# rockcarry/ffcnn

Measured on AMD Instinct MI355X. Metric: frames/sec yolo-fastest-1.1 @320x320 batch-64 per GPU (u8 BGR frames -> net_input's conversion in the first kernel -> full forward: conv stack + YOLO decode + NMS, boxes on rank 0), higher is better.
Workload: dtype f32

## Files before the change

ffcnn_amd/capi.py:

```python
import ctypes as C
import os
import subprocess

import numpy as np

HERE = os.path.dirname(os.path.abspath(__file__))
ROOT = os.path.dirname(HERE)
DATA = os.path.join(ROOT, "data")
CFG = os.path.join(DATA, "yolo-fastest-1.1.cfg")
WEIGHTS = os.path.join(DATA, "yolo-fastest-1.1.weights")

f32p = C.POINTER(C.c_float)


class FFGPU:
    MAX_DET = 128
    MERGE_LDS_SLOTS = 1024
    KEEP_ALL, COMPAT_V6, NO_GRAPH, NO_FUSE, HOST_DETS, SPLIT2, CONCURRENT, BF16_PW = 1, 2, 4, 8, 16, 32, 64, 128
    FEAT_FLAT, FEAT_MEAN, FEAT_MAX = 0, 1, 2
    POST_NONE, POST_SOFTMAX, POST_L2 = 0, 1, 2
    TOPK_MAX = 16
    RELABEL_KEEP_SCORE, RELABEL_LABEL_SCORE = 0, 1
    RELABEL_ENTRIES, RELABEL_MERGED = 0, 1
    K_AUTO, K_GENERIC, K_DW_STREAM, K_DW_LDS, K_PW_MFMA, K_PW_GEMM, _K6, K_DENSE_SMALL, K_IGEMM, K_PW_BF16, K_GROUP_THIN, K_PW_X3, K_CONV_X3, K_PW_X3T = range(14)
# ... 264 lines not shown
TRAIL_SLOT_DTYPE = np.dtype([("id", "<i4"), ("last", "<i4"), ("n", "<i4"), ("head", "<i4"), ("cx", "<i4"), ("cy", "<i4"), ("reserved", "<i4", (2,)),
                             ("ring", TRAIL_POINT_DTYPE, (32,))])
LABEL_DTYPE = np.dtype([("index", "<i4"), ("value", "<f4")])
TEXT_ITEM_DTYPE = np.dtype([("x", "<i4"), ("y", "<i4"), ("fg", "u1", (4,)), ("bg", "u1", (4,)), ("scale", "u1"), ("flags", "u1"), ("len", "u1"), ("reserved", "u1"),
                            ("text", "u1", (44,))])
SEG_ITEM_DTYPE = np.dtype([("x0", "<i4"), ("y0", "<i4"), ("x1", "<i4"), ("y1", "<i4"), ("color", "u1", (4,)), ("thickness", "u1"), ("dash", "u1"), ("flags", "u1"),
                           ("reserved", "u1"), ("reserved2", "<i4", (2,))])

EXPORTS = ["net_load", "net_free", "net_input", "net_forward", "net_dump", "net_profile", "groupconv",
           "ffgpu_device_count", "ffgpu_set_device", "ffgpu_last_error", "ffgpu_build_info",
           "ffgpu_net_weights_dev", "ffgpu_net_weights_commit",
           "ffgpu_exec_create", "ffgpu_exec_destroy", "ffgpu_exec_batch", "ffgpu_exec_arena_bytes",
           "ffgpu_exec_kernel_count", "ffgpu_exec_work_model", "ffgpu_exec_set_scale", "ffgpu_exec_forward_dev", "ffgpu_exec_forward_host",
           "ffgpu_exec_forward_bgr_dev", "ffgpu_exec_forward_bgr_frames_dev", "ffgpu_exec_forward_nv12_frames_dev", "ffgpu_exec_dets_dev", "ffgpu_exec_dets_host", "ffgpu_exec_set_ring", "ffgpu_exec_set_ring_strided", "ffgpu_exec_read_dets", "ffgpu_exec_read_layer", "ffgpu_exec_hash_layers",
           "ffgpu_exec_read_boxes", "ffgpu_exec_cand_capacity", "ffgpu_exec_graph_captures",
           "ffgpu_exec_profile", "ffgpu_exec_profile_steps", "ffgpu_exec_step_model", "ffgpu_groupconv_dev", "ffgpu_groupconv_kernel_name", "ffgpu_groupconv_time_dev", "ffgpu_irb_dev", "ffgpu_irb_flags_dev", "ffgpu_irb_plan_text", "ffgpu_irb_thin_launch_text", "ffgpu_irb_stage_plan_text", "ffgpu_front_plan_text", "ffgpu_irb_instantiations", "ffgpu_knobs_text", "ffgpu_dwpw_dev", "ffgpu_packed_records_bytes", "ffgpu_pack_records", "ffgpu_unpack_records",
           "ffgpu_shard_range", "ffgpu_node_create", "ffgpu_node_destroy", "ffgpu_node_ndev", "ffgpu_node_shard", "ffgpu_node_set_scale",
           "ffgpu_node_input_dev", "ffgpu_node_input_slot_dev", "ffgpu_node_depth", "ffgpu_node_rccl_ranks", "ffgpu_node_forward", "ffgpu_node_forward_host",
           "ffgpu_node_submit", "ffgpu_node_wait", "ffgpu_node_run",
           "ffgpu_merge_tiles_scratch_bytes", "ffgpu_merge_tiles_dev", "ffgpu_exec_merge_tiles", "ffgpu_exec_merged_dev", "ffgpu_exec_read_merged",
           "ffgpu_exec_read_merged_boxes", "ffgpu_tile_plan",
           "ffgpu_draw_boxes_bgr_dev", "ffgpu_draw_boxes_nv12_dev", "ffgpu_exec_draw_bgr", "ffgpu_exec_draw_nv12",
           "ffgpu_crop_table_bytes", "ffgpu_crop_slot_bytes", "ffgpu_crop_boxes_bgr_dev", "ffgpu_crop_boxes_nv12_dev", "ffgpu_exec_crop_bgr", "ffgpu_exec_crop_nv12",
           "ffgpu_crops_to_source_dev",
           "ffgpu_track_state_bytes", "ffgpu_track_reset_dev", "ffgpu_track_boxes_dev", "ffgpu_exec_track",
           "ffgpu_feature_dim", "ffgpu_exec_feature_dim", "ffgpu_features_dev", "ffgpu_exec_features", "ffgpu_topk_dev", "ffgpu_crops_relabel_dev",
           "ffgpu_exec_relabel",
           "ffgpu_match_workspace_bytes", "ffgpu_match_dev", "ffgpu_gallery_enroll_dev",
           "ffgpu_redact_boxes_bgr_dev", "ffgpu_redact_boxes_nv12_dev", "ffgpu_exec_redact_bgr", "ffgpu_exec_redact_nv12",
           "ffgpu_blur_boxes_bgr_dev", "ffgpu_blur_boxes_nv12_dev", "ffgpu_exec_blur_bgr", "ffgpu_exec_blur_nv12",
           "ffgpu_zones_state_bytes", "ffgpu_scene_check", "ffgpu_zones_reset_dev", "ffgpu_zones_boxes_dev", "ffgpu_exec_zones",
# ... 73 lines not shown
    L.ffgpu_exec_read_layer.argtypes = [vp, i, i, f32p, sz]
    L.ffgpu_exec_hash_layers.argtypes = [vp, vp, i]
    L.ffgpu_exec_profile.argtypes = [vp, vp, f32p]
    L.ffgpu_exec_profile_steps.argtypes = [vp, vp, C.POINTER(i), f32p, i]
    L.ffgpu_exec_step_model.argtypes = [vp, C.POINTER(i), C.POINTER(C.c_double), i]
    L.ffgpu_groupconv_dev.argtypes = [vp, vp, vp] + [i] * 15 + [vp]
    L.ffgpu_groupconv_kernel_name.restype = C.c_char_p
    L.ffgpu_groupconv_kernel_name.argtypes = [i] * 10
    L.ffgpu_groupconv_time_dev.restype = C.c_float
    L.ffgpu_groupconv_time_dev.argtypes = [vp, vp, vp] + [i] * 17 + [vp]
    L.ffgpu_irb_dev.restype = C.c_float
    L.ffgpu_irb_dev.argtypes = [vp] * 6 + [i] * 13 + [vp]
    L.ffgpu_irb_flags_dev.restype = C.c_float
    L.ffgpu_irb_flags_dev.argtypes = [vp] * 6 + [i] * 14 + [vp]
    L.ffgpu_irb_thin_launch_text.argtypes = [i] * 12 + [C.c_char_p, i]
    L.ffgpu_irb_plan_text.argtypes = [i] * 12 + [C.c_char_p, i]
    L.ffgpu_irb_stage_plan_text.argtypes = [i] * 7 + [C.c_char_p, i]
    L.ffgpu_front_plan_text.argtypes = [i] * 4 + [C.c_char_p, i]
    L.ffgpu_irb_instantiations.argtypes = [C.c_char_p, i]
    L.ffgpu_knobs_text.argtypes = [C.c_char_p, i]
    L.ffgpu_exec_read_boxes.argtypes = [vp, i, vp, i]
    L.ffgpu_exec_cand_capacity.argtypes = [vp]
    L.ffgpu_exec_graph_captures.argtypes = [vp]
    L.ffgpu_dwpw_dev.restype = C.c_float
    L.ffgpu_dwpw_dev.argtypes = [vp] * 4 + [i] * 10 + [vp]
    L.ffgpu_packed_records_bytes.restype = C.c_size_t
    L.ffgpu_packed_records_bytes.argtypes = [i, i]
    L.ffgpu_pack_records.restype = i
    L.ffgpu_pack_records.argtypes = [vp, i, C.c_long, i, i, vp, vp]
    L.ffgpu_shard_range.argtypes = [i, i, i, C.POINTER(i), C.POINTER(i)]
# ... 1308 lines not shown

def dwpw_dev(d_in, d_wd, d_wp, d_out, batch, iw, ih, c, oc, fs, actd=2, actp=0, warmup=0, iters=0, stream=None):
    us = lib().ffgpu_dwpw_dev(d_in, d_wd, d_wp, d_out, batch, iw, ih, c, oc, fs, actd, actp, warmup, iters, stream)
    if us < 0:
        raise RuntimeError("ffgpu_dwpw_dev failed: %s" % last_error())
    return us


def irb_thin_launch_text(shape, flags=0):
    buf = C.create_string_buffer(256)
    if lib().ffgpu_irb_thin_launch_text(*shape, flags, buf, len(buf)) < 0:
        raise RuntimeError("ffgpu_irb_thin_launch_text failed: %s" % last_error())
    return buf.value.decode()


def irb_dev(d_in, d_w1, d_wd, d_w2, d_res, d_out, batch, iw, ih, ic, ec, oc, stride, act1=2, actd=2, act2=0, res_act=0,
            warmup=0, iters=0, stream=None, flags=0):
    us = lib().ffgpu_irb_flags_dev(d_in, d_w1, d_wd, d_w2, d_res, d_out, batch, iw, ih, ic, ec, oc, stride, act1, actd, act2, res_act, flags,
                                   warmup, iters, stream)
    if us < 0:
        raise RuntimeError("ffgpu_irb_dev failed: %s" % last_error())
    return us


def preview_pane(src=None, dst=None):
    p = PreviewPane()
    if src is not None:
        p.sx, p.sy, p.sw, p.sh = (int(v) for v in src)
    if dst is not None:
        p.dx, p.dy, p.dw, p.dh = (int(v) for v in dst)
# ... 139 lines not shown
```

ffcnn_amd/csrc/ffgpu_conv_kernels.inc:

```
#include "ffgpu_dw_stream.inc"
#include "ffgpu_pw_mfma.inc"
#include "ffgpu_pw_gemm32.inc"
#include "ffgpu_pw_bf16.inc"
#include "ffgpu_conv_igemm.inc"
#include "ffgpu_dwpw.inc"
#include "ffgpu_conv_dense.inc"
#include "ffgpu_irb.inc"
#include "ffgpu_irb_thin.inc"
#include "ffgpu_front.inc"
#include "ffgpu_irb_wave.inc"
#include "ffgpu_irb_wave2.inc"
#include "ffgpu_irb_stage.inc"
#include "ffgpu_pw_x3.inc"
#include "ffgpu_pw_x3t.inc"
#include "ffgpu_conv_x3.inc"
#include "ffgpu_dw_lds.inc"
#include "ffgpu_dw_pair.inc"
#include "ffgpu_conv_thin.inc"

struct BareScratch {
    float *p = nullptr; size_t n = 0; int dev = -1;
    float *get(size_t need)
    {
        int d = 0;
// ... 1040 lines not shown
    if (f.ncp) { p.band = f.band; p.nbands = f.nbands; p.ntasks = f.ntasks; }
    for (const IrbThinKernel &k : irb_thin_kernels)
        if (k.IC == d.ic && k.OC == d.oc) return f.ncp ? k.pair(p, f, s) : k.launch(p, d.plan, s);
    ffgpu_set_error("irb_thin: no instantiation for %d -> 8 -> %d channels", d.ic, d.oc);
    return -1;
}

int ffgpu_irb_thin_launch_line(const IrbDesc &d, char *buf, size_t cap)
{
    if (d.plan.family != IRB_THIN) return snprintf(buf, cap, "unsupported");
    const ThinForm f = thin_form(d);
    char key[48];
    if (f.ncp) snprintf(key, sizeof key, "thin_pair<%d,8,%d,%d>", d.ic, d.oc, f.ncp);
    else snprintf(key, sizeof key, "thin<%d,8,%d>", d.ic, d.oc);
    return snprintf(buf, cap, "%s W=%d H=%d N=%d band=%d nbands=%d ntasks=%ld grid=%d block=256", key, d.W, d.H, d.N, f.band, f.nbands, f.ntasks, f.grid);
}

typedef int (*IrbwLaunch)(const IrbwP &, const IrbPlan &, hipStream_t);
struct IrbwKernel { int KS1, OT, S, NSI, NSO; bool big, x3, xl; Knob gate; IrbwLaunch launch; };
#define IRBW_K(ks1, ot, st, nsi, gate) \
    { ks1, ot, st, nsi, 1, true, false, false, gate, irb_launch_t<IrbwP, k_irbw<ks1, ot, st, nsi, true>> }, \
    { ks1, ot, st, nsi, 1, false, false, false, gate, irb_launch_t<IrbwP, k_irbw<ks1, ot, st, nsi, false>> }
static const IrbwKernel irbw_kernels[] = {
    { 2, 1, 1, 3, 2, true, true, false, K_NONE, irb_launch_t<IrbwP, k_irbw2<2, 3, true>> }, { 4, 1, 1, 3, 2, true, true, false, K_NONE, irb_launch_t<IrbwP, k_irbw2<4, 3, true>> },
    { 2, 1, 1, 3, 2, true, false, false, K_NONE, irb_launch_t<IrbwP, k_irbw2<2, 3, false>> }, { 4, 1, 1, 3, 2, true, false, false, K_NONE, irb_launch_t<IrbwP, k_irbw2<4, 3, false>> },
    { 12, 3, 1, 2, 1, true, true, true, K_NONE, irb_launch_t<IrbwP, k_irbw<12, 3, 1, 2, true, true, true>> },
    { 4, 2, 2, 4, 1, true, true, false, K_NONE, irb_launch_t<IrbwP, k_irbw<4, 2, 2, 4, true, true>> },
    { 6, 2, 1, 2, 1, true, true, false, K_NONE, irb_launch_t<IrbwP, k_irbw<6, 2, 1, 2, true, true>> },
    IRBW_K(1, 1, 1, 2, K_NONE), IRBW_K(2, 1, 1, 2, K_NONE), IRBW_K(4, 1, 1, 2, K_NONE), IRBW_K(2, 2, 1, 2, K_NONE), IRBW_K(4, 2, 1, 2, K_NONE),
    IRBW_K(6, 2, 1, 2, K_NONE), IRBW_K(12, 3, 1, 2, K_NONE), IRBW_K(1, 1, 2, 3, K_NONE), IRBW_K(2, 1, 2, 3, K_NONE), IRBW_K(4, 2, 2, 4, K_NONE),
// ... 480 lines not shown
                        key, p.N, p.H, p.W, p.OH, p.OW, p.ic, p.ec, p.oc, p.act1, p.actd, p.act2, p.res_act, p.TWq, p.TH, p.EW, p.EH, p.tiles_x, p.tiles_y, p.ntiles, p.ngroups, p.G, p.WPB,
                        p.o_w2, p.o_cs, p.cs_floats, p.xl_off, p.red_cap, p.in_elems, p.vec, p.half_last, p.m_ew, p.m_tx, p.m_ty, p.m_twq, p.xcd, c.lds, c.grid, c.block, c.half, c.pack_floats);
    }
    if (c.family == IRB_WG) {
        const IrbP p = irb_params(d);
        const IrbKernel &k = irb_kernels[c.inst];
        irb_key(k, key, sizeof key);
        return snprintf(buf, cap, "%s N=%d H=%d W=%d OH=%d OW=%d ic=%d ec=%d oc=%d stride=%d act=%g,%g,%g,%g tile=%d,%d,%d,%d,%d,%d NPin=%d NPout=%d tiles=%d,%d,%d "
                        "k4=%d nchunks=%d ECH=%d CH=%d KS=%d red_off=%d vec_store=%d resident=%d inv_nsi=%d lds=%d grid=%d block=%d half=%d pack=%d",
                        key, p.N, p.H, p.W, p.OH, p.OW, p.ic, p.ec, p.oc, p.stride, p.act1, p.actd, p.act2, p.res_act, p.TH, p.TW, p.TWq, p.NF, p.EH, p.EW,
                        p.NPin, p.NPout, p.tiles_x, p.tiles_y, p.ntiles, p.k4, p.nchunks, p.ECH, p.CH, p.KS, p.red_off, p.vec_store, p.resident, p.inv_nsi, c.lds, c.grid, c.block, c.half, c.pack_floats);
    }
    return snprintf(buf, cap, "unsupported");
}

int ffgpu_launch_irb(const IrbDesc &d, hipStream_t s)
{
    const IrbPlan &c = d.plan;
    if (!irb_planned(d, "irb")) return -1;
    if (knob(K_VERBOSE_IRB)) { char line[1024]; ffgpu_irb_plan_line(d, line, sizeof line); fprintf(stderr, "%s\n", line); }
    if (c.family == IRB_THIN) return launch_irb_thin(d, s);
    if (!d.pk) { ffgpu_set_error("irb: constants not packed"); return -1; }
    return c.family == IRB_WAVE ? irbw_kernels[c.inst].launch(irbw_params(d), c, s) : irb_kernels[c.inst].launch(irb_params(d), c, s);
}

static bool irb_stage_params(const IrbDesc *blocks, int B, IrbStageP &p, size_t &lds)
{
    if (B < 2 || B > IRBS_MAXB) return false;
    const IrbDesc &d0 = blocks[0];
    for (int b = 0; b < B; b++) {
        const IrbDesc &d = blocks[b];
        const IrbPlan &c = d.plan;
        if (d.ic != 48 || d.ec != 224 || d.oc != 48 || d.stride != 1 || d.OH != d.H || d.OW != d.W) return false;
        if (d.N != d0.N || d.H != d0.H || d.W != d0.W || d.act1 != d0.act1 || d.actd != d0.actd) return false;
        if (act_slope(d.act2) != 1.f || act_slope(d.res_act) != 1.f) return false;
        if (c.family != IRB_WAVE || !c.xl || !c.x3 || c.half || c.G != IRBS_WAVES || c.KS1 != 12 || c.OT != 3 || c.ngroups != 2 * IRBS_WAVES) return false;
// ... 50 lines not shown
```

ffcnn_amd/csrc/ffgpu_dev.hpp:

```cpp
#pragma once
#include <hip/hip_runtime.h>
#include <stddef.h>
#include <stdint.h>
#include <vector>
#include "ffgpu_internal.h"
#include "ffgpu_args.hpp"
#include "ffgpu_streams_host.hpp"
#include "ffgpu_track_host.hpp"
#include "ffgpu_zones_host.hpp"
#include "ffgpu_text_host.hpp"
#include "ffgpu_lines_host.hpp"
#include "ffgpu_trails_host.hpp"
#include "ffgpu_heat_host.hpp"
#include "ffgpu_motion_host.hpp"
#include "ffgpu_preview_host.hpp"
#include "ffgpu_warp_host.hpp"

#define FFGPU_CHECK(expr)                                                                   \
    do {                                                                                    \
        hipError_t e_ = (expr);                                                             \
        if (e_ != hipSuccess) {                                                             \
            ffgpu_set_error("%s failed: %s (%s:%d)", #expr, hipGetErrorString(e_), __FILE__, __LINE__); \
            return -1;                                                                      \
        }                                                                                   \
// ... 37 lines not shown
struct IrbDesc {
    const float *in; float *out; const float *residual;
    const float *w1, *wd, *w2;
    int N, H, W, OH, OW, ic, ec, oc, stride;
    int act1, actd, act2, res_act;
    const float *pk;
    int flags;
    IrbPlan plan;
};
bool   ffgpu_irb_plan(IrbDesc &d);
size_t ffgpu_irb_pack_floats(const IrbDesc &d);
int    ffgpu_irb_pack(const IrbDesc &d, float *pk, hipStream_t s);
int    ffgpu_launch_irb(const IrbDesc &d, hipStream_t s);
int    ffgpu_irb_plan_line(const IrbDesc &d, char *buf, size_t cap);
int    ffgpu_irb_thin_launch_line(const IrbDesc &d, char *buf, size_t cap);
int    ffgpu_irb_keys(char *buf, size_t cap);
#define IRBS_MAXB 8
bool   ffgpu_irb_stage_ok(const IrbDesc *blocks, int B);
int    ffgpu_launch_irb_stage(const IrbDesc *blocks, int B, hipStream_t s);
int    ffgpu_irb_stage_line(const IrbDesc *blocks, int B, bool wanted, char *buf, size_t cap);
bool   ffgpu_front_ok(const ConvDesc &c, const IrbDesc &d);
enum InputForm { IN_F32, IN_U8, IN_BGR_FRAMES, IN_NV12_FRAMES, IN_FORMS };
int    ffgpu_launch_front(const ConvDesc &c, const IrbDesc &d, InputForm form, hipStream_t s);
bool   ffgpu_front_nv12_fused();
int    ffgpu_front_plan_line(const IrbDesc &d, InputForm form, char *buf, size_t cap);
int    ffgpu_front_nc(const IrbDesc &d);

bool   ffgpu_dwpw_ok(const ConvDesc &dw, const ConvDesc &pw);
size_t ffgpu_dwpw_pack_floats(const ConvDesc &dw, const ConvDesc &pw);
int    ffgpu_dwpw_pack(const ConvDesc &dw, const ConvDesc &pw, float *pk, hipStream_t s);
// ... 117 lines not shown
```

ffcnn_amd/csrc/ffgpu_exec.hip:

```cpp
#include <algorithm>
#include <cstdarg>
#include <cstdint>
#include <cstdio>
#include <cstdlib>
#include <cstring>
#include <map>
#include <mutex>
#include <string>
#include <type_traits>
#include <vector>

#include "ffgpu_dev.hpp"
#include "ffgpu_knobs.hpp"
#include "ffgpu_plan.hpp"
#include "conv.h"

static thread_local char g_err[512] = "";

extern "C" void ffgpu_set_error(const char *fmt, ...)
{
    va_list ap;
    va_start(ap, fmt);
    vsnprintf(g_err, sizeof g_err, fmt, ap);
    va_end(ap);
// ... 1812 lines not shown
{
    if (!buf || cap < 1) { ffgpu_set_error("knobs_text: bad arguments"); return -1; }
    return ffgpu_knobs_lines(buf, (size_t)cap);
}

extern "C" int ffgpu_irb_thin_launch_text(int batch, int iw, int ih, int ic, int ec, int oc, int stride, int act1, int actd, int act2, int res_act, int flags, char *buf, int cap)
{
    if (!buf || cap < 1 || batch < 1 || iw < 1 || ih < 1 || stride < 1) { ffgpu_set_error("irb_thin_launch_text: bad arguments"); return -1; }
    IrbDesc d{};
    irb_fill(d, batch, iw, ih, ic, ec, oc, stride, act1, actd, act2, res_act);
    d.flags = flags & FFGPU_CONCURRENT;
    (void)ffgpu_irb_plan(d);
    return ffgpu_irb_thin_launch_line(d, buf, (size_t)cap);
}

extern "C" float ffgpu_irb_dev(const float *d_in, const float *d_w1, const float *d_wd, const float *d_w2,
                               const float *d_res, float *d_out, int batch, int iw, int ih, int ic, int ec, int oc,
                               int stride, int act1, int actd, int act2, int res_act, int warmup, int iters, void *stream)
{
    return ffgpu_irb_flags_dev(d_in, d_w1, d_wd, d_w2, d_res, d_out, batch, iw, ih, ic, ec, oc, stride, act1, actd, act2, res_act, 0, warmup, iters, stream);
}

extern "C" float ffgpu_irb_flags_dev(const float *d_in, const float *d_w1, const float *d_wd, const float *d_w2,
                                     const float *d_res, float *d_out, int batch, int iw, int ih, int ic, int ec, int oc,
                                     int stride, int act1, int actd, int act2, int res_act, int flags, int warmup, int iters, void *stream)
{
    hipStream_t s = (hipStream_t)stream;
    IrbDesc d{};
    d.in = d_in; d.out = d_out; d.residual = d_res; d.w1 = d_w1; d.wd = d_wd; d.w2 = d_w2;
    irb_fill(d, batch, iw, ih, ic, ec, oc, stride, act1, actd, act2, res_act);
// ... 94 lines not shown
```

ffcnn_amd/csrc/ffgpu_knobs.hpp:

```cpp
#pragma once
#include <assert.h>
#include <limits.h>
#include <stdio.h>
#include <stdlib.h>

enum KnobKind { KNOB_INT, KNOB_ON, KNOB_SET, KNOB_TEXT };
enum KnobClass { KNOB_PRODUCT, KNOB_TUNING, KNOB_TEST, KNOB_LAB };
#define KNOB_COMPUTED INT_MIN

#define FFGPU_KNOBS_MAIN(X) \
     \
    X(COMPAT_V6,         "FFCNN_COMPAT_V6",         ON,   0,             PRODUCT, "the reference's v6 behaviour for 5x5 filters (executors and groupconv)") \
    X(NO_GRAPH,          "FFGPU_NO_GRAPH",          ON,   0,             PRODUCT, "eager launches instead of a captured graph (as the flag FFGPU_NO_GRAPH)") \
    X(BF16_PW,           "FFGPU_BF16_PW",           ON,   0,             PRODUCT, "opt-in bf16 inputs for compute-bound pointwise layers; own tolerance (as the flag)") \
    X(NO_FUSE,           "FFGPU_NO_FUSE",           ON,   0,             PRODUCT, "one kernel per layer: no fused blocks, no concat in place, no residual in the conv epilogue (as the flag)") \
    X(BRANCH,            "FFGPU_BRANCH",            ON,   0,             PRODUCT, "first detection head as a parallel graph branch instead of in line") \
    X(DWPW,              "FFGPU_DWPW",              ON,   0,             PRODUCT, "the heads' depthwise + pointwise pairs as one kernel (measured slower)") \
    X(NO_U8_FRONT,       "FFGPU_NO_U8_FRONT",       SET,  0,             PRODUCT, "u8 frames through the staging kernel and the fp32 first kernel even where they could go straight in") \
    X(NV12_FRONT,        "FFGPU_NV12_FRONT",        INT,  KNOB_COMPUTED, PRODUCT, "1: NV12 frames into the NV12 form of k_front where the plan has it, 0: staged; default: the build's measured choice") \
    X(VERBOSE,           "FFGPU_VERBOSE",           SET,  0,             PRODUCT, "print every error to stderr as it is set") \
    X(NODE_PACK_BOXES,   "FFGPU_NODE_PACK_BOXES",   INT,  0,             PRODUCT, "room per frame in a shard's packed record block; 0 or less: 16, the constant of the same name in ffgpu_node.inc") \
    X(NO_IRB,            "FFGPU_NO_IRB",            ON,   0,             TUNING,  "no fused inverted-residual blocks: their three layers as three kernels") \
    X(IRB_MIN_EC,        "FFGPU_IRB_MIN_EC",        INT,  24,            TUNING,  "fewest expanded channels of a block the planner fuses (thin blocks apart)") \
    X(IRB_STAGE,         "FFGPU_IRB_STAGE",         INT,  1,             TUNING,  "runs of 48 -> 224 -> 48 blocks on a small plane as one launch in FFGPU_CONCURRENT executors of 32 frames or more (0: one launch per block)") \
// ... 40 lines not shown
    X(IGEMM_SPLIT,       "FFGPU_IGEMM_SPLIT",       INT,  0,             TUNING,  "k_conv_igemm: split-K factor 1 .. 16 (0: by tile count; frozen with a plan: ConvDesc::nsplit)") \
    X(DW_U,              "FFGPU_DW_U",              INT,  4,             TUNING,  "k_dw3_stream: rows per step, 1 / 2 / 4") \
    X(DW_BAND,           "FFGPU_DW_BAND",           INT,  4,             TUNING,  "k_dw3_stream: rows per wave task (0: enough tasks to fill the chip)") \
    X(DW_NT,             "FFGPU_DW_NT",             INT,  -1,            PRODUCT, "k_dw3_stream: stream past the caches never (0) / always (1); -1: outputs of 128 MB and more") \
    X(DW_XCD,            "FFGPU_DW_XCD",            INT,  0,             TUNING,  "k_dw3_stream: walk the tasks XCD by XCD") \
    X(DWP_NI,            "FFGPU_DWP_NI",            INT,  0,             TUNING,  "k_dw_pair: frames per workgroup, at most (0: by shape)") \
    X(DWL_BH,            "FFGPU_DWL_BH",            INT,  0,             TUNING,  "k_dw_lds: rows per band (0: by shape)") \
    X(DWL_NPL,           "FFGPU_DWL_NPL",           INT,  0,             TUNING,  "k_dw_lds: planes per item (0: by shape)") \
    X(PWG_WM,            "FFGPU_PWG_WM",            INT,  0,             TUNING,  "k_pw_gemm32: waves per workgroup, 4 or 8 (0: 8 from 248 output channels; part of the packed image)") \
    X(PWG_NARROW,        "FFGPU_PWG_NARROW",        INT,  1,             TUNING,  "k_pw_gemm32: 0 switches the narrow tiles of the partial last round off") \
    X(PWG_DBG,           "FFGPU_PWG_DBG",           INT,  0,             LAB,     "k_pw_gemm32: ablation mask handed to the kernel (wrong results)") \
     \
    X(NO_THIN,           "FFGPU_NO_THIN",           INT,  0,             PRODUCT, "8-channel blocks on the wave kernel instead of k_irb_thin") \
    X(THIN_BAND,         "FFGPU_THIN_BAND",         INT,  KNOB_COMPUTED, TUNING,  "k_irb_thin: rows per wave; default by batch and height (thin_band)") \
    X(THIN_PAIR,         "FFGPU_THIN_PAIR",         INT,  1,             TUNING,  "k_irb_thin: 0 keeps FFGPU_CONCURRENT executors off the paired form (two frames per wave, 3 / 4 / 5 columns per lane); read at launch") \
    X(FRONT_BAND,        "FFGPU_FRONT_BAND",       INT,  KNOB_COMPUTED, TUNING,  "k_front: rows per wave; default as FFGPU_THIN_BAND") \
    X(NO_FRONT,          "FFGPU_NO_FRONT",          INT,  0,             PRODUCT, "layers 0-3 as k_conv_first + k_irb_thin instead of k_front") \
    X(FRONT_MIN_PX,      "FFGPU_FRONT_MIN_PX",      INT,  262144,        TUNING,  "k_front: fewest output pixels of the batch") \
    X(FRONT_NC,          "FFGPU_FRONT_NC",          INT,  3,             PRODUCT, "k_front: output columns per lane, 3 where a row fits a wave that way, or 4") \
    X(NO_IRBW,           "FFGPU_NO_IRBW",           INT,  0,             PRODUCT, "fused blocks on the workgroup kernel k_irb instead of the wave-autonomous k_irbw") \
    X(IRBW_S2_633,       "FFGPU_IRBW_S2_633",       INT,  1,             TUNING,  "k_irbw: 0 hides the stride-2 form for 24 input / 48 output channels from the planner") \
    X(IRBW_S2_NSI4,      "FFGPU_IRBW_S2_NSI4",      INT,  0,             TUNING,  "k_irbw: 1 lets the planner take the four-strip halo for the thin stride-2 blocks") \
    X(IRBW_TWQ,          "FFGPU_IRBW_TWQ",          INT,  0,             TUNING,  "k_irbw: tile width in quads (with FFGPU_IRBW_TH; 0: searched)") \
    X(IRBW_TH,           "FFGPU_IRBW_TH",           INT,  0,             TUNING,  "k_irbw: tile height (with FFGPU_IRBW_TWQ; 0: searched)") \
    X(IRBW_BIG,          "FFGPU_IRBW_BIG",          INT,  -1,            TUNING,  "k_irbw: the 256-register form never (0) / always (1); -1: by register need") \
    X(IRBW_BIG_S2K1,     "FFGPU_IRBW_BIG_S2K1",     INT,  -1,            TUNING,  "k_irbw: as FFGPU_IRBW_BIG for the stride-2 blocks of at most 4 input channels alone") \
    X(IRBW_GWAVES,       "FFGPU_IRBW_GWAVES",       INT,  KNOB_COMPUTED, TUNING,  "k_irbw: waves a launch wants before the group split stops; default 1200, 500 with FFGPU_CONCURRENT") \
    X(IRBW_NOEXC,        "FFGPU_IRBW_NOEXC",        INT,  0,             TUNING,  "k_irbw: without the measured exception (four waves on the 20x20 blocks)") \
    X(IRBW_G_MID,        "FFGPU_IRBW_G_MID",        INT,  0,             TUNING,  "k_irbw: group split for 256 .. 1099 tiles (0: as computed)") \
    X(IRBW_X3,           "FFGPU_IRBW_X3",           INT,  30,            PRODUCT, "fused blocks: expand GEMM as split-bf16 products, one bit per shape: 0: 8 input channels, 1: 16, 2: 24, 3: 48 (split tile in LDS), 4: the 40 -> 20 stride-2 block") \
// ... 84 lines not shown
```

include/ffcnn_hip.h:

```cpp
#ifndef FFCNN_AMD_FFCNN_HIP_H
#define FFCNN_AMD_FFCNN_HIP_H

#include <stddef.h>
#include "ffcnn.h"

#ifdef __cplusplus
extern "C" {
#endif

#define FFGPU_MAX_DET   128



typedef struct {
    int  count;
    int  ncand;
    int  overflow;
    int  nfull;
    BBOX box[FFGPU_MAX_DET];
} ffgpu_frame_dets;

typedef struct ffgpu_exec ffgpu_exec;

#define FFGPU_KEEP_ALL   1
// ... 125 lines not shown
                               int iw, int ih, int ic, int groups, int pad, int stride,
                               int fs, int fn, int ow, int oh, int oc, int act,
                               int flags, int variant, int warmup, int iters, void *stream);

float ffgpu_irb_dev(const float *d_in, const float *d_w1, const float *d_wd, const float *d_w2,
                    const float *d_res, float *d_out, int batch, int iw, int ih, int ic, int ec, int oc,
                    int stride, int act1, int actd, int act2, int res_act, int warmup, int iters, void *stream);

float ffgpu_irb_flags_dev(const float *d_in, const float *d_w1, const float *d_wd, const float *d_w2,
                          const float *d_res, float *d_out, int batch, int iw, int ih, int ic, int ec, int oc,
                          int stride, int act1, int actd, int act2, int res_act, int flags, int warmup, int iters, void *stream);

int ffgpu_irb_thin_launch_text(int batch, int iw, int ih, int ic, int ec, int oc, int stride, int act1, int actd, int act2, int res_act,
                               int flags, char *buf, int cap);

int ffgpu_irb_plan_text(int batch, int iw, int ih, int ic, int ec, int oc, int stride, int act1, int actd, int act2, int res_act,
                        int flags, char *buf, int cap);

int ffgpu_irb_stage_plan_text(int batch, int iw, int ih, int blocks, int act1, int actd, int flags, char *buf, int cap);

int ffgpu_front_plan_text(int batch, int pw, int ph, int form, char *buf, int cap);

int ffgpu_irb_instantiations(char *buf, int cap);

int ffgpu_knobs_text(char *buf, int cap);

float ffgpu_dwpw_dev(const float *d_in, const float *d_wd, const float *d_wp, float *d_out, int batch, int iw, int ih,
                     int c, int oc, int fs, int actd, int actp, int warmup, int iters, void *stream);

size_t ffgpu_packed_records_bytes(int batch, int cap);
// ... 570 lines not shown
```

Before: 209,300.

## Add streaming thin kernel for stride-2 4->24->8 inverted residual block

Adds k_irb_thin_s2, a row-streaming fused expand/depthwise-stride-2/project kernel for the 4->24->8 block. It keeps weights in LDS, uses packed two-channel math and DPP neighbour shifts, and processes several frames per wave in row bands. It is selected over the planned wave kernel when the executor runs with FFGPU_CONCURRENT. This aims to cut the LDS tiling overhead of the generic kernel on this thin layer, at the cost of a new code path and halo recompute at band edges.

After: 215,600 (median of 6 runs). +3.0%, better.

```diff
diff --git a/ffcnn_amd/capi.py b/ffcnn_amd/capi.py
--- a/ffcnn_amd/capi.py
+++ b/ffcnn_amd/capi.py
@@ -302,7 +302,7 @@
            "ffgpu_exec_kernel_count", "ffgpu_exec_work_model", "ffgpu_exec_set_scale", "ffgpu_exec_forward_dev", "ffgpu_exec_forward_host",
            "ffgpu_exec_forward_bgr_dev", "ffgpu_exec_forward_bgr_frames_dev", "ffgpu_exec_forward_nv12_frames_dev", "ffgpu_exec_dets_dev", "ffgpu_exec_dets_host", "ffgpu_exec_set_ring", "ffgpu_exec_set_ring_strided", "ffgpu_exec_read_dets", "ffgpu_exec_read_layer", "ffgpu_exec_hash_layers",
            "ffgpu_exec_read_boxes", "ffgpu_exec_cand_capacity", "ffgpu_exec_graph_captures",
-           "ffgpu_exec_profile", "ffgpu_exec_profile_steps", "ffgpu_exec_step_model", "ffgpu_groupconv_dev", "ffgpu_groupconv_kernel_name", "ffgpu_groupconv_time_dev", "ffgpu_irb_dev", "ffgpu_irb_flags_dev", "ffgpu_irb_plan_text", "ffgpu_irb_thin_launch_text", "ffgpu_irb_stage_plan_text", "ffgpu_front_plan_text", "ffgpu_irb_instantiations", "ffgpu_knobs_text", "ffgpu_dwpw_dev", "ffgpu_packed_records_bytes", "ffgpu_pack_records", "ffgpu_unpack_records",
+           "ffgpu_exec_profile", "ffgpu_exec_profile_steps", "ffgpu_exec_step_model", "ffgpu_groupconv_dev", "ffgpu_groupconv_kernel_name", "ffgpu_groupconv_time_dev", "ffgpu_irb_dev", "ffgpu_irb_flags_dev", "ffgpu_irb_plan_text", "ffgpu_irb_thin_launch_text", "ffgpu_irb_s2_launch_text", "ffgpu_irb_stage_plan_text", "ffgpu_front_plan_text", "ffgpu_irb_instantiations", "ffgpu_knobs_text", "ffgpu_dwpw_dev", "ffgpu_packed_records_bytes", "ffgpu_pack_records", "ffgpu_unpack_records",
            "ffgpu_shard_range", "ffgpu_node_create", "ffgpu_node_destroy", "ffgpu_node_ndev", "ffgpu_node_shard", "ffgpu_node_set_scale",
            "ffgpu_node_input_dev", "ffgpu_node_input_slot_dev", "ffgpu_node_depth", "ffgpu_node_rccl_ranks", "ffgpu_node_forward", "ffgpu_node_forward_host",
            "ffgpu_node_submit", "ffgpu_node_wait", "ffgpu_node_run",
@@ -406,6 +406,7 @@
     L.ffgpu_irb_flags_dev.restype = C.c_float
     L.ffgpu_irb_flags_dev.argtypes = [vp] * 6 + [i] * 14 + [vp]
     L.ffgpu_irb_thin_launch_text.argtypes = [i] * 12 + [C.c_char_p, i]
+    L.ffgpu_irb_s2_launch_text.argtypes = [i] * 12 + [C.c_char_p, i]
     L.ffgpu_irb_plan_text.argtypes = [i] * 12 + [C.c_char_p, i]
     L.ffgpu_irb_stage_plan_text.argtypes = [i] * 7 + [C.c_char_p, i]
     L.ffgpu_front_plan_text.argtypes = [i] * 4 + [C.c_char_p, i]
@@ -1744,6 +1745,13 @@
     return buf.value.decode()
 
 
+def irb_s2_launch_text(shape, flags=0):
+    buf = C.create_string_buffer(256)
+    if lib().ffgpu_irb_s2_launch_text(*shape, flags, buf, len(buf)) < 0:
+        raise RuntimeError("ffgpu_irb_s2_launch_text failed: %s" % last_error())
+    return buf.value.decode()
+
+
 def irb_dev(d_in, d_w1, d_wd, d_w2, d_res, d_out, batch, iw, ih, ic, ec, oc, stride, act1=2, actd=2, act2=0, res_act=0,
             warmup=0, iters=0, stream=None, flags=0):
     us = lib().ffgpu_irb_flags_dev(d_in, d_w1, d_wd, d_w2, d_res, d_out, batch, iw, ih, ic, ec, oc, stride, act1, actd, act2, res_act, flags,
diff --git a/ffcnn_amd/csrc/ffgpu_conv_kernels.inc b/ffcnn_amd/csrc/ffgpu_conv_kernels.inc
--- a/ffcnn_amd/csrc/ffgpu_conv_kernels.inc
+++ b/ffcnn_amd/csrc/ffgpu_conv_kernels.inc
@@ -7,6 +7,7 @@
 #include "ffgpu_conv_dense.inc"
 #include "ffgpu_irb.inc"
 #include "ffgpu_irb_thin.inc"
+#include "ffgpu_irb_thin_s2.inc"
 #include "ffgpu_front.inc"
 #include "ffgpu_irb_wave.inc"
 #include "ffgpu_irb_wave2.inc"
@@ -1078,6 +1079,44 @@
     if (f.ncp) snprintf(key, sizeof key, "thin_pair<%d,8,%d,%d>", d.ic, d.oc, f.ncp);
     else snprintf(key, sizeof key, "thin<%d,8,%d>", d.ic, d.oc);
     return snprintf(buf, cap, "%s W=%d H=%d N=%d band=%d nbands=%d ntasks=%ld grid=%d block=256", key, d.W, d.H, d.N, f.band, f.nbands, f.ntasks, f.grid);
+}
+
+#define THIN_S2_NC 3
+#define THIN_S2_WAVES 640
+struct ThinS2Form { bool on; int lpr, F, band, nbands; long ntasks; int grid; };
+static ThinS2Form thin_s2_form(const IrbDesc &d)
+{
+    ThinS2Form f{};
+    const int lpr = (d.OW + THIN_S2_NC - 1) / THIN_S2_NC;
+    f.on = d.stride == 2 && d.ic == 4 && d.ec == 24 && d.oc == 8 && d.W % 2 == 0 && d.OW == d.W / 2 && d.OH == (d.H + 1) / 2 && d.OW >= THIN_S2_NC && lpr <= 32 &&
+           d.N >= 2 && (d.flags & FFGPU_CONCURRENT) && !d.residual &&
+           (size_t)d.ic * d.N * d.H * d.W < (1u << 30) &&
+           d.act1 != 3 && d.actd != 3 && d.act2 != 3 && knob(K_THIN_S2) != 0;
+    if (!f.on) return f;
+    f.lpr = lpr; f.F = 64 / lpr;
+    const int groups = (d.N + f.F - 1) / f.F;
+    int band = 2;
+    while (band < 16 && (long)groups * d.OH >= (long)THIN_S2_WAVES * band * 2) band *= 2;
+    if (const int kb = knob(K_THIN_S2_BAND); kb > 0) band = kb;
+    f.band = band;
+    f.nbands = (d.OH + f.band - 1) / f.band;
+    f.ntasks = (long)groups * f.nbands;
+    f.grid = (int)((f.ntasks + 3) / 4);
+    return f;
+}
+
+static int launch_irb_thin_s2(const IrbDesc &d, const ThinS2Form &f, hipStream_t s)
+{
+    ThinS2P p;
+    p.in = d.in; p.out = d.out; p.w1 = d.w1; p.wd = d.wd; p.w2 = d.w2;
+    p.W = d.W; p.H = d.H; p.N = d.N; p.OW = d.OW; p.OH = d.OH;
+    p.lpr = f.lpr; p.F = f.F; p.band = f.band; p.nbands = f.nbands;
+    p.act1 = act_slope(d.act1); p.actd = act_slope(d.actd); p.act2 = act_slope(d.act2);
+    p.ntasks = f.ntasks;
+    if (!p.in || !p.out || !p.w1 || !p.wd || !p.w2) { ffgpu_set_error("irb_thin_s2: no tensors or filter rows"); return -1; }
+    hipLaunchKernelGGL((k_irb_thin_s2<4, 24, 8, THIN_S2_NC>), dim3((unsigned)f.grid), dim3(256), 0, s, p);
+    LAUNCH_OK("irb_thin_s2");
+    return 0;
 }
 
 typedef int (*IrbwLaunch)(const IrbwP &, const IrbPlan &, hipStream_t);
@@ -1588,12 +1627,32 @@
     return snprintf(buf, cap, "unsupported");
 }
 
+int ffgpu_irb_s2_launch_line(const IrbDesc &d, char *buf, size_t cap)
+{
+    const IrbPlan &c = d.plan;
+    char key[48];
+    if (c.family == IRB_NONE) return snprintf(buf, cap, "unsupported");
+    if (c.family == IRB_THIN) {
+        const ThinP p = thin_params(d);
+        irb_thin_key(d.ic, d.oc, key, sizeof key);
+        return snprintf(buf, cap, "%s frames=1 band=%d tasks=%ld grid=%d block=%d", key, p.band, p.ntasks, c.grid, c.block);
+    }
+    if (const ThinS2Form f = thin_s2_form(d); f.on)
+        return snprintf(buf, cap, "thin_s2<%d,%d,%d,%d> frames=%d band=%d tasks=%ld grid=%d block=256 W=%d H=%d N=%d lanes=%d nbands=%d",
+                        d.ic, d.ec, d.oc, THIN_S2_NC, f.F, f.band, f.ntasks, f.grid, d.W, d.H, d.N, f.lpr, f.nbands);
+    long tiles;
+    if (c.family == IRB_WAVE) { irbw_key(irbw_kernels[c.inst], key, sizeof key); tiles = irbw_params(d).ntiles; }
+    else { irb_key(irb_kernels[c.inst], key, sizeof key); tiles = irb_params(d).ntiles; }
+    return snprintf(buf, cap, "%s frames=%d band=%d tasks=%ld grid=%d block=%d", key, c.family == IRB_WG ? c.NF : 1, c.TH, tiles, c.grid, c.block);
+}
+
 int ffgpu_launch_irb(const IrbDesc &d, hipStream_t s)
 {
     const IrbPlan &c = d.plan;
     if (!irb_planned(d, "irb")) return -1;
     if (knob(K_VERBOSE_IRB)) { char line[1024]; ffgpu_irb_plan_line(d, line, sizeof line); fprintf(stderr, "%s\n", line); }
     if (c.family == IRB_THIN) return launch_irb_thin(d, s);
+    if (const ThinS2Form f = thin_s2_form(d); f.on) return launch_irb_thin_s2(d, f, s);
     if (!d.pk) { ffgpu_set_error("irb: constants not packed"); return -1; }
     return c.family == IRB_WAVE ? irbw_kernels[c.inst].launch(irbw_params(d), c, s) : irb_kernels[c.inst].launch(irb_params(d), c, s);
 }
diff --git a/ffcnn_amd/csrc/ffgpu_dev.hpp b/ffcnn_amd/csrc/ffgpu_dev.hpp
--- a/ffcnn_amd/csrc/ffgpu_dev.hpp
+++ b/ffcnn_amd/csrc/ffgpu_dev.hpp
@@ -75,6 +75,7 @@
 int    ffgpu_launch_irb(const IrbDesc &d, hipStream_t s);
 int    ffgpu_irb_plan_line(const IrbDesc &d, char *buf, size_t cap);
 int    ffgpu_irb_thin_launch_line(const IrbDesc &d, char *buf, size_t cap);
+int    ffgpu_irb_s2_launch_line(const IrbDesc &d, char *buf, size_t cap);
 int    ffgpu_irb_keys(char *buf, size_t cap);
 #define IRBS_MAXB 8
 bool   ffgpu_irb_stage_ok(const IrbDesc *blocks, int B);
diff --git a/ffcnn_amd/csrc/ffgpu_exec.hip b/ffcnn_amd/csrc/ffgpu_exec.hip
--- a/ffcnn_amd/csrc/ffgpu_exec.hip
+++ b/ffcnn_amd/csrc/ffgpu_exec.hip
@@ -1850,6 +1850,16 @@
     return ffgpu_irb_thin_launch_line(d, buf, (size_t)cap);
 }
 
+extern "C" int ffgpu_irb_s2_launch_text(int batch, int iw, int ih, int ic, int ec, int oc, int stride, int act1, int actd, int act2, int res_act, int flags, char *buf, int cap)
+{
+    if (!buf || cap < 1 || batch < 1 || iw < 1 || ih < 1 || stride < 1) { ffgpu_set_error("irb_s2_launch_text: bad arguments"); return -1; }
+    IrbDesc d{};
+    irb_fill(d, batch, iw, ih, ic, ec, oc, stride, act1, actd, act2, res_act);
+    d.flags = flags & FFGPU_CONCURRENT;
+    (void)ffgpu_irb_plan(d);
+    return ffgpu_irb_s2_launch_line(d, buf, (size_t)cap);
+}
+
 extern "C" float ffgpu_irb_dev(const float *d_in, const float *d_w1, const float *d_wd, const float *d_w2,
                                const float *d_res, float *d_out, int batch, int iw, int ih, int ic, int ec, int oc,
                                int stride, int act1, int actd, int act2, int res_act, int warmup, int iters, void *stream)
diff --git a/ffcnn_amd/csrc/ffgpu_irb_thin_s2.inc b/ffcnn_amd/csrc/ffgpu_irb_thin_s2.inc
--- /dev/null
+++ b/ffcnn_amd/csrc/ffgpu_irb_thin_s2.inc
@@ -0,0 +1,225 @@
+struct ThinS2P {
+    const float *in; float *out;
+    const float *w1, *wd, *w2;
+    int W, H, N, OW, OH;
+    int lpr, F;
+    int band, nbands;
+    float act1, actd, act2;
+    long ntasks;
+};
+
+template <int IC, int EC, int OC, int NC>
+__global__ void __launch_bounds__(256) __attribute__((amdgpu_waves_per_eu(2))) k_irb_thin_s2(ThinS2P p)
+{
+    static_assert(EC % 2 == 0 && OC % 2 == 0, "channel pairs");
+    static_assert(NC >= 2 && NC <= 4, "columns per lane");
+    constexpr int K4 = (IC + 3) & ~3, RL1 = K4 + 4, RL2 = ((EC + 3) & ~3) + 4, OCP = (OC + 3) & ~3, CP = EC / 2, NI = 2 * NC;
+    constexpr int T1 = (IC + 2) * 2, TE = 8, TO = 16, T2 = 2 * OCP;
+    static_assert(T1 % 4 == 0 && T2 % 4 == 0, "16-byte table reads");
+    __shared__ __attribute__((aligned(16))) float tw[CP * (T1 + TE + TO + T2) + 2 * OCP];
+    float *t1 = tw, *te = tw + CP * T1, *to = te + CP * TE, *t2 = to + CP * TO, *tsb = t2 + CP * T2;
+    for (int i = threadIdx.x; i < CP * T1; i += 256) {
+        const int cp = i / T1, j = (i % T1) >> 1, c = 2 * cp + (i & 1);
+        t1[i] = p.w1[c * RL1 + (j < IC ? j : K4 + (j - IC))];
+    }
+    for (int i = threadIdx.x; i < CP * TE; i += 256) {
+        const int cp = i / TE, j = (i % TE) >> 1, c = 2 * cp + (i & 1);
+        te[i] = j < 3 ? p.wd[c * 16 + 3 + j] : 0.f;
+    }
+    for (int i = threadIdx.x; i < CP * TO; i += 256) {
+        const int cp = i / TO, j = (i % TO) >> 1, c = 2 * cp + (i & 1);
+        to[i] = p.wd[c * 16 + (j < 3 ? 6 + j : (j < 5 ? 9 + j : j - 5))];
+    }
+    for (int i = threadIdx.x; i < CP * T2; i += 256) {
+        const int cp = i / T2, h = (i % T2) / OCP, k = i % OCP;
+        t2[i] = k < OC ? p.w2[k * RL2 + 2 * cp + h] : 0.f;
+    }
+    for (int i = threadIdx.x; i < 2 * OCP; i += 256) { const int k = i % OCP; tsb[i] = k < OC ? p.w2[k * RL2 + RL2 - 4 + i / OCP] : 0.f; }
+    __syncthreads();
+    const int lane = threadIdx.x & 63;
+    const int task = blockIdx.x * 4 + __builtin_amdgcn_readfirstlane(threadIdx.x >> 6);
+    if (task >= p.ntasks) return;
+    const int g = task / p.nbands, band_i = task - g * p.nbands;
+    const int slot = lane / p.lpr, hl = lane - slot * p.lpr;
+    const bool have = slot < p.F && g * p.F + slot < p.N;
+    const bool first_col = hl == 0, last_col = hl == p.lpr - 1;
+    const int sl = p.lpr * NC - p.OW;
+    const int x0 = last_col ? p.OW - NC : hl * NC;
+    const int n = have ? g * p.F + slot : g * p.F;
+    const unsigned HW = (unsigned)p.W * p.H, OHW = (unsigned)p.OW * p.OH;
+    const unsigned cs = (unsigned)p.N * HW, ocs = (unsigned)p.N * OHW;
+    const unsigned lo = (unsigned)n * HW + 2u * x0, oo = (unsigned)n * OHW + x0;
+    const int y0 = band_i * p.band, y1 = min(y0 + p.band, p.OH);
+    typedef float v2f_s2 __attribute__((ext_vector_type(2)));
+    const v2f_s2 z2 = { 0.f, 0.f };
+
+    typedef float v4a4 __attribute__((ext_vector_type(4), aligned(4)));
+    typedef float v3a4 __attribute__((ext_vector_type(3), aligned(4)));
+    typedef float v2a4 __attribute__((ext_vector_type(2), aligned(4)));
+    struct Row { float c[IC][NI]; };
+    auto load_row = [&](int r, Row &x) __attribute__((always_inline)) {
+        const unsigned ro = (unsigned)min(max(r, 0), p.H - 1) * p.W + lo;
+#pragma unroll
+        for (int ci = 0; ci < IC; ci++) {
+            const float *src = p.in + (ci * cs + ro);
+            const v4a4 a = *reinterpret_cast<const v4a4 *>(src);
+            x.c[ci][0] = a.x; x.c[ci][1] = a.y; x.c[ci][2] = a.z; x.c[ci][3] = a.w;
+            if constexpr (NC == 3) { const v2a4 b = *reinterpret_cast<const v2a4 *>(src + 4); x.c[ci][4] = b.x; x.c[ci][5] = b.y; }
+            if constexpr (NC == 4) { const v4a4 b = *reinterpret_cast<const v4a4 *>(src + 4); x.c[ci][4] = b.x; x.c[ci][5] = b.y; x.c[ci][6] = b.z; x.c[ci][7] = b.w; }
+        }
+    };
+    struct W1T { v4f q[T1 / 4]; };
+    struct WET { v4f q[TE / 4]; };
+    struct WOT { v4f q[TO / 4]; v4f w2[T2 / 4]; };
+    auto ld1 = [&](int cp) { W1T r;
+#pragma unroll
+        for (int j = 0; j < T1 / 4; j++) r.q[j] = *reinterpret_cast<const v4f *>(t1 + cp * T1 + 4 * j);
+        return r; };
+    auto lde = [&](int cp) { WET r;
+#pragma unroll
+        for (int j = 0; j < TE / 4; j++) r.q[j] = *reinterpret_cast<const v4f *>(te + cp * TE + 4 * j);
+        return r; };
+    auto ldo = [&](int cp) { WOT r;
+#pragma unroll
+        for (int j = 0; j < TO / 4; j++) r.q[j] = *reinterpret_cast<const v4f *>(to + cp * TO + 4 * j);
+#pragma unroll
+        for (int j = 0; j < T2 / 4; j++) r.w2[j] = *reinterpret_cast<const v4f *>(t2 + cp * T2 + 4 * j);
+        return r; };
+
+    v2f_s2 S[CP][NC];
+    Row X[2];
+#pragma unroll
+    for (int c = 0; c < CP; c++)
+#pragma unroll
+        for (int j = 0; j < NC; j++) S[c][j] = z2;
+    load_row(2 * y0 - 1, X[0]);
+
+    auto step = [&](int r, auto PAR) {
+        constexpr bool ODD = decltype(PAR)::value != 0;
+        asm volatile("" ::: "memory");
+        const bool rin = r >= 0 && r < p.H, fin = ODD && r > 2 * y0;
+        const Row &x = X[ODD ? 0 : 1];
+        if (r < 2 * y1 - 1) load_row(r + 1, X[ODD ? 1 : 0]);
+        v2f_s2 o[OCP / 2][NC];
+        if constexpr (ODD) {
+#pragma unroll
+            for (int k = 0; k < OCP / 2; k++)
+#pragma unroll
+                for (int j = 0; j < NC; j++) o[k][j] = z2;
+        }
+        W1T n1 = ld1(0);
+        __builtin_amdgcn_sched_barrier(0);
+#pragma unroll
+        for (int cp = 0; cp < CP; cp++) {
+            const W1T c1 = n1;
+            WET ce; WOT co;
+            if constexpr (ODD) co = ldo(cp); else ce = lde(cp);
+            __builtin_amdgcn_sched_barrier(0);
+            auto w1p = [&](int j) { return (j & 1) ? (v2f_s2){ c1.q[j >> 1].z, c1.q[j >> 1].w } : (v2f_s2){ c1.q[j >> 1].x, c1.q[j >> 1].y }; };
+            auto wep = [&](int j) { return (j & 1) ? (v2f_s2){ ce.q[j >> 1].z, ce.q[j >> 1].w } : (v2f_s2){ ce.q[j >> 1].x, ce.q[j >> 1].y }; };
+            auto wop = [&](int j) { return (j & 1) ? (v2f_s2){ co.q[j >> 1].z, co.q[j >> 1].w } : (v2f_s2){ co.q[j >> 1].x, co.q[j >> 1].y }; };
+            v2f_s2 win[NI + 1];
+            if (rin) {
+#pragma unroll
+                for (int j = 0; j < NI; j++) {
+                    v2f_s2 a = w1p(0) * x.c[0][j];
+#pragma unroll
+                    for (int ci = 1; ci < IC; ci++) a += w1p(ci) * x.c[ci][j];
+                    a = a * w1p(IC) + w1p(IC + 1);
+                    const v2f_s2 u = a * p.act1;
+                    win[1 + j] = (v2f_s2){ act_max(a.x, u.x, act_floor(p.act1)), act_max(a.y, u.y, act_floor(p.act1)) };
+                }
+            } else {
+#pragma unroll
+                for (int j = 0; j < NI; j++) win[1 + j] = z2;
+            }
+            if (cp + 1 < CP) n1 = ld1(cp + 1);
+            win[0] = (v2f_s2){ dpp_shr1(win[NI].x), dpp_shr1(win[NI].y) };
+            if (sl) {
+                v2f_s2 src = win[NI - 2];
+#pragma unroll
+                for (int k = 2; k < NC; k++) if (sl == k) src = win[NI - 2 * k];
+                const v2f_s2 alt = { dpp_shr1(src.x), dpp_shr1(src.y) };
+                win[0] = (v2f_s2){ last_col ? alt.x : win[0].x, last_col ? alt.y : win[0].y };
+            }
+            win[0] = (v2f_s2){ first_col ? 0.f : win[0].x, first_col ? 0.f : win[0].y };
+            __builtin_amdgcn_sched_barrier(0);
+            if constexpr (!ODD) {
+#pragma unroll
+                for (int j = 0; j < NC; j++) {
+                    v2f_s2 m = S[cp][j];
+                    m += wep(0) * win[2 * j]; m += wep(1) * win[2 * j + 1]; m += wep(2) * win[2 * j + 2];
+                    S[cp][j] = m;
+                }
+            } else {
+                if (fin) {
+#pragma unroll
+                    for (int j = 0; j < NC; j++) {
+                        v2f_s2 d = S[cp][j];
+                        d += wop(0) * win[2 * j]; d += wop(1) * win[2 * j + 1]; d += wop(2) * win[2 * j + 2];
+                        d = d * wop(3) + wop(4);
+                        const v2f_s2 u = d * p.actd;
+                        d = (v2f_s2){ act_max(d.x, u.x, act_floor(p.actd)), act_max(d.y, u.y, act_floor(p.actd)) };
+#pragma unroll
+                        for (int k = 0; k < OCP / 2; k++) {
+                            const v4f &wa = co.w2[k >> 1], &wb = co.w2[(OCP / 2 + k) >> 1];
+                            const v2f_s2 w2a = (k & 1) ? (v2f_s2){ wa.z, wa.w } : (v2f_s2){ wa.x, wa.y };
+                            const v2f_s2 w2b = ((OCP / 2 + k) & 1) ? (v2f_s2){ wb.z, wb.w } : (v2f_s2){ wb.x, wb.y };
+                            o[k][j] += w2a * d.x;
+                            o[k][j] += w2b * d.y;
+                        }
+                    }
+                }
+#pragma unroll
+                for (int j = 0; j < NC; j++) {
+                    v2f_s2 s = wop(5) * win[2 * j];
+                    s += wop(6) * win[2 * j + 1]; s += wop(7) * win[2 * j + 2];
+                    S[cp][j] = s;
+                }
+            }
+#pragma unroll
+            for (int j = 0; j < NC; j++) asm volatile("" : "+v"(S[cp][j]));
+            if constexpr (ODD) {
+                if (fin) {
+#pragma unroll
+                    for (int k = 0; k < OCP / 2; k++)
+#pragma unroll
+                        for (int j = 0; j < NC; j++) asm volatile("" : "+v"(o[k][j]));
+                }
+            }
+            __builtin_amdgcn_sched_barrier(0);
+        }
+        if constexpr (ODD) {
+            if (fin && have) {
+                v4f sb[2 * OCP / 4];
+#pragma unroll
+                for (int j = 0; j < 2 * OCP / 4; j++) sb[j] = *reinterpret_cast<const v4f *>(tsb + 4 * j);
+                const unsigned orow = (unsigned)((r - 1) >> 1) * p.OW + oo;
+#pragma unroll
+                for (int k = 0; k < OC / 2; k++) {
+                    const v4f &sq = sb[k >> 1], &bq = sb[(OCP / 2 + k) >> 1];
+                    const v2f_s2 sc = (k & 1) ? (v2f_s2){ sq.z, sq.w } : (v2f_s2){ sq.x, sq.y };
+                    const v2f_s2 bi = ((OCP / 2 + k) & 1) ? (v2f_s2){ bq.z, bq.w } : (v2f_s2){ bq.x, bq.y };
+                    v2f_s2 v[4];
+#pragma unroll
+                    for (int j = 0; j < NC; j++) {
+                        const v2f_s2 t = o[k][j] * sc + bi, u = t * p.act2;
+                        v[j] = (v2f_s2){ act_max(t.x, u.x, act_floor(p.act2)), act_max(t.y, u.y, act_floor(p.act2)) };
+                    }
+#pragma unroll
+                    for (int h = 0; h < 2; h++) {
+                        float *dst = p.out + ((2 * k + h) * ocs + orow);
+                        if constexpr (NC == 2) *reinterpret_cast<v2a4 *>(dst) = (v2a4){ v[0][h], v[1][h] };
+                        else if constexpr (NC == 3) *reinterpret_cast<v3a4 *>(dst) = (v3a4){ v[0][h], v[1][h], v[2][h] };
+                        else *reinterpret_cast<v4a4 *>(dst) = (v4a4){ v[0][h], v[1][h], v[2][h], v[3][h] };
+                    }
+                }
+            }
+        }
+    };
+    step(2 * y0 - 1, std::integral_constant<int, 1>());
+    for (int y = y0; y < y1; y++) {
+        step(2 * y, std::integral_constant<int, 0>());
+        step(2 * y + 1, std::integral_constant<int, 1>());
+    }
+}
diff --git a/ffcnn_amd/csrc/ffgpu_knobs.hpp b/ffcnn_amd/csrc/ffgpu_knobs.hpp
--- a/ffcnn_amd/csrc/ffgpu_knobs.hpp
+++ b/ffcnn_amd/csrc/ffgpu_knobs.hpp
@@ -78,6 +78,8 @@
     X(NO_THIN,           "FFGPU_NO_THIN",           INT,  0,             PRODUCT, "8-channel blocks on the wave kernel instead of k_irb_thin") \
     X(THIN_BAND,         "FFGPU_THIN_BAND",         INT,  KNOB_COMPUTED, TUNING,  "k_irb_thin: rows per wave; default by batch and height (thin_band)") \
     X(THIN_PAIR,         "FFGPU_THIN_PAIR",         INT,  1,             TUNING,  "k_irb_thin: 0 keeps FFGPU_CONCURRENT executors off the paired form (two frames per wave, 3 / 4 / 5 columns per lane); read at launch") \
+    X(THIN_S2,           "FFGPU_THIN_S2",           INT,  1,             TUNING,  "k_irb_thin_s2: 0 keeps FFGPU_CONCURRENT executors off the streaming form of the stride-2 block 4 -> 24 -> 8 (the planned wave kernel instead); read at launch") \
+    X(THIN_S2_BAND,      "FFGPU_THIN_S2_BAND",      INT,  0,             TUNING,  "k_irb_thin_s2: output rows per wave (0: by batch and height, thin_s2_form); read at launch") \
     X(FRONT_BAND,        "FFGPU_FRONT_BAND",       INT,  KNOB_COMPUTED, TUNING,  "k_front: rows per wave; default as FFGPU_THIN_BAND") \
     X(NO_FRONT,          "FFGPU_NO_FRONT",          INT,  0,             PRODUCT, "layers 0-3 as k_conv_first + k_irb_thin instead of k_front") \
     X(FRONT_MIN_PX,      "FFGPU_FRONT_MIN_PX",      INT,  262144,        TUNING,  "k_front: fewest output pixels of the batch") \
diff --git a/include/ffcnn_hip.h b/include/ffcnn_hip.h
--- a/include/ffcnn_hip.h
+++ b/include/ffcnn_hip.h
@@ -163,6 +163,9 @@
 int ffgpu_irb_thin_launch_text(int batch, int iw, int ih, int ic, int ec, int oc, int stride, int act1, int actd, int act2, int res_act,
                                int flags, char *buf, int cap);
 
+int ffgpu_irb_s2_launch_text(int batch, int iw, int ih, int ic, int ec, int oc, int stride, int act1, int actd, int act2, int res_act,
+                             int flags, char *buf, int cap);
+
 int ffgpu_irb_plan_text(int batch, int iw, int ih, int ic, int ec, int oc, int stride, int act1, int actd, int act2, int res_act,
                         int flags, char *buf, int cap);
 
```
